# AiRyunn/BoT

Hardware: AMD Instinct MI355X
Metric: edges/sec full-batch GAT fwd+bwd on ogbn-arxiv; achieved HBM GB/s vs peak (higher is better)
Workload: dtype f32

## Files before the change

### bot_amd/_C.py

```python
from __future__ import annotations

import ctypes
import os
from ctypes import c_char_p, c_double, c_float, c_int32, c_int64, c_uint64, c_void_p

import torch

_HERE = os.path.dirname(os.path.abspath(__file__))
LIB_PATH = os.environ.get("BOT_AMD_LIB") or os.path.join(_HERE, "lib", "libbot_gnn.so")
ABI_VERSION = 19

if not os.path.exists(LIB_PATH):
    raise ImportError(
        f"{LIB_PATH} is missing: build the gfx950 kernels first "
        "(`make -C bot_amd/csrc` or `python -c 'import __graft_entry__ as g; g.build()'`). "
        "bot_amd has no CPU / PyTorch fallback."
    )
_lib = ctypes.CDLL(LIB_PATH)

_P = c_void_p
_SIGS = {
    "bot_abi_version": (ctypes.c_int, []),
    "bot_last_error": (c_char_p, []),
    "bot_last_kernel": (c_char_p, []),
# ... 32 lines not shown
    "bot_segment_sum_f32": (ctypes.c_int, [_P, c_int64, c_int64, _P, c_int64, c_int32, _P, _P, c_int32, _P, _P]),
    "bot_gather_rows_f32": (ctypes.c_int, [_P, c_int64, _P, c_int64, c_int32, _P, c_int64, _P]),
    "bot_scatter_add_rows_f32": (ctypes.c_int, [_P, c_int64, _P, c_int64, c_int32, _P, c_int64, _P]),
    "bot_merge_weight_fwd_f32": (ctypes.c_int, [_P, _P, _P, _P, c_int32, c_int32, c_int32, c_int32, c_int32, c_int32, _P, _P]),
    "bot_merge_weight_bwd_f32": (ctypes.c_int, [_P, _P, _P, c_int32, c_int32, c_int32, c_int32, c_int32, c_int32, _P, _P, _P, _P, _P, _P]),
    "bot_edge_mlp_workspace_floats": (c_int64, []),
    "bot_edge_mlp_fwd_f32": (ctypes.c_int, [_P, c_int32, _P, _P, c_int32, _P, c_int32, c_int64, _P, _P]),
    "bot_edge_mlp_bwd_f32": (ctypes.c_int, [_P, c_int32, _P, _P, c_int32, _P, c_int32, _P, c_int64, _P, _P, _P, _P, _P]),
    "bot_random_keep_workspace_bytes": (c_int64, []),
    "bot_random_keep_u8": (ctypes.c_int, [c_int64, c_int64, c_uint64, _P, _P, _P]),
    "bot_halves_workspace_floats": (c_int64, []),
    "bot_halves_scale_f32": (ctypes.c_int, [_P, c_int64, c_int64, c_int32, _P, _P, _P]),
    "bot_halves_split_f16": (ctypes.c_int, [_P, c_int64, c_int64, c_int32, _P, c_int32, _P, c_int64, c_int32, _P]),
    "bot_halves_split_cols_f16": (ctypes.c_int, [_P, c_int64, c_int64, c_int32, _P, c_int32, _P, c_int64, c_int32, c_int32, _P]),
    "bot_halves_split_heads_f16": (ctypes.c_int, [_P, c_int64, c_int64, c_int32, c_int32, _P, _P, c_int64, c_int32, c_int32, _P]),
    "bot_gemm_halves_f32": (ctypes.c_int, [c_int32, c_int32, c_int64, c_int64, c_int64, _P, _P, c_int64, _P, c_int64, _P, c_int64,
                                           c_int32, c_int64, c_int64, c_int64, c_float, _P, c_int64, c_int32, c_int32, _P]),
    "bot_gemm_halves3_nt_f32": (ctypes.c_int, [c_int64, c_int64, c_int64, _P, _P, _P, c_int64, c_int64, _P, c_int64, c_int64, _P, c_int64,
                                               c_int32, _P]),
    "bot_gemm_halves3_tn_workspace_floats": (c_int64, [c_int64, c_int64, c_int64]),
    "bot_gemm_halves3_tn_f32": (ctypes.c_int, [c_int64, c_int64, c_int64, c_int64, c_int64, _P, _P, _P, c_int64, c_int64, _P, c_int64, c_int64, _P,
                                               c_int64, _P, c_int32, _P]),
    "bot_gemm_halves3_nt_grouped_f32": (ctypes.c_int, [c_int64, c_int64, _P, _P, _P, c_int64, c_int64, _P, c_int64, c_int64, _P, c_int64, c_int32, _P,
                                                       c_int32, _P, _P, c_int32, _P, c_int32, _P]),
    "bot_gemm_halves3_tn_grouped_workspace_floats": (c_int64, [c_int64, c_int32]),
    "bot_gemm_halves3_tn_grouped_f32": (ctypes.c_int, [c_int64, _P, _P, _P, c_int64, c_int64, _P, c_int64, c_int64, _P, c_int32, _P, _P, c_int32, _P]),
    "bot_tn_narrow_workspace_floats": (c_int64, [c_int64, c_int32, c_int32]),
    "bot_tn_narrow_f32": (ctypes.c_int, [_P, c_int64, _P, c_int64, c_int64, c_int32, c_int32, _P, c_int64, c_int32, _P, _P]),
    "bot_bn_act_bwd_reduce_max_f32": (ctypes.c_int, [_P, c_int64, _P, c_int64, c_int64, c_int32, _P, _P, _P, _P, c_int32, c_float, c_uint64, _P, _P, _P, _P, _P]),
    "bot_bn_bwd_bound_f32": (ctypes.c_int, [c_int32, c_int64, _P, _P, _P, c_double, _P, _P, _P, _P]),
    "bot_bn_act_bwd_apply_halves_f32": (ctypes.c_int, [_P, c_int64, _P, c_int64, c_int64, c_int32, _P, _P, _P, _P, c_int32, c_float, c_uint64, _P, _P, _P, c_double,
                                                       _P, c_int64, _P, _P, c_int64, c_int32, c_int32, c_int32, _P]),
    "bot_label_split_f32": (ctypes.c_int, [_P, c_int64, _P, c_int64, _P, c_float, c_uint64, _P, c_int32, _P, _P, _P, _P, _P]),
    "bot_build_input_f32": (ctypes.c_int, [_P, c_int64, c_int64, c_int32, c_int32, _P, c_float, c_uint64, _P, _P, c_int64, _P]),
    "bot_node_loss_f32": (ctypes.c_int, [_P, c_int64, c_int64, c_int32, _P, c_int64, _P, _P, c_int32, c_float, _P, c_int64, _P, c_int64, _P]),
    "bot_rmsprop_step_f32": (ctypes.c_int, [c_int32, _P, _P, _P, _P, c_float, _P, c_float, c_float, c_float, _P]),
    "bot_gemm_halves_last_algo": (ctypes.c_int, [_P, _P]),
    "bot_gemm_halves_library_version": (ctypes.c_int, [_P, _P]),
    "bot_tn_gemm_workspace_floats": (c_int64, [c_int64, c_int32, c_int32, c_int32]),
    "bot_tn_gemm_f32": (ctypes.c_int, [_P, c_int64, _P, c_int64, c_int64, c_int32, c_int32, _P, c_int64, c_int32, c_int32, c_int64, c_int64,
                                       c_int64, _P, _P]),
    "bot_skinny_gemm_f32": (ctypes.c_int, [_P, c_int64, _P, c_int64, c_int32, _P, c_int64, c_int64, c_int32, c_int32, c_int32, c_int32,
                                           c_int64, c_int64, c_int64, _P]),
    "bot_bn_workspace_floats": (c_int64, [c_int32]),
    "bot_colstats_f32": (ctypes.c_int, [_P, c_int64, c_int64, c_int32, _P, _P, _P, _P]),
    "bot_colsum_f32": (ctypes.c_int, [_P, c_int64, c_int64, c_int32, _P, _P, _P]),
    "bot_bn_stats_f32": (ctypes.c_int, [_P, c_int64, c_int64, c_int32, c_float, c_float, _P, _P, _P, _P, _P, _P, _P]),
    "bot_bn_stats_halves_f32": (ctypes.c_int, [_P, c_int64, c_int64, c_int32, c_float, c_float, _P, _P, _P, _P, _P, _P, _P, c_float, _P, _P, _P]),
    "bot_bn_act_fwd_halves_f32": (ctypes.c_int, [_P, c_int64, c_int64, c_int32, _P, _P, _P, _P, c_int32, c_float, c_uint64, _P, _P, c_int64,
                                                 _P, _P, c_int64, c_int32, c_int32, _P]),
    "bot_bn_act_fwd_f32": (ctypes.c_int, [_P, c_int64, c_int64, c_int32, _P, _P, _P, _P, c_int32, c_float, c_uint64, _P, _P, c_int64, _P]),
    "bot_bn_act_bwd_reduce_f32": (ctypes.c_int, [_P, c_int64, _P, c_int64, c_int64, c_int32, _P, _P, _P, _P, c_int32, c_float,
                                                 c_uint64, _P, _P, _P, _P, _P]),
    "bot_bn_act_bwd_apply_f32": (ctypes.c_int, [_P, c_int64, _P, c_int64, c_int64, c_int32, _P, _P, _P, _P, c_int32, c_float,
                                                c_uint64, _P, _P, _P, c_double, _P, c_int64, _P, _P]),
    "bot_halves_tn_combine_f32": (ctypes.c_int, [_P, _P, c_int32, c_int32, c_int32, c_int32, _P, _P, _P, c_int64, _P]),
    "bot_halves_scale_from_slots2_f32": (ctypes.c_int, [_P, c_float, _P, c_float, _P, _P]),
    "bot_halves_tail_f16": (ctypes.c_int, [c_int64, c_int32, _P, _P, _P, _P, _P, c_int64, c_int32, _P]),
    "bot_spmm_dot_halves_fits": (ctypes.c_int, [_P, c_int64, c_int64, _P, c_int64, c_int64, c_int32, c_int32, _P, c_int64, c_int64, c_int32]),
    "bot_spmm_dot_halves_f16": (ctypes.c_int, [_P, _P, c_int64, c_int64, _P, c_int64, _P, _P, c_int64, _P, c_int64, c_int64, _P, _P, _P, c_int64, c_int64,
                                               c_int32, c_int32, _P, _P, c_int64, c_int64, c_int32, _P, _P, _P]),
    "bot_gemm_halves3_nt_bn_rows": (c_int32, [c_int64]),
    "bot_gemm_halves3_nt3_f32": (ctypes.c_int, [c_int64, c_int64, c_int64, _P, _P, c_int64, _P, _P, c_int64, c_int64, _P, c_int64, c_int64, c_int32, _P, c_int64,
                                                _P, c_int32, _P]),
    "bot_bn_act_bwd_reduce_partials_f32": (ctypes.c_int, [_P, c_int32, c_int32, _P, _P, _P]),
    "bot_bn_bwd_bound_partials_f32": (ctypes.c_int, [c_int32, _P, c_int32, _P, _P, c_double, _P, _P, _P, _P]),
    "bot_bn_bwd_partials_finish_f32": (ctypes.c_int, [_P, _P, c_int32, c_int32, _P, _P, c_int32, c_double, _P, _P, _P, _P]),
    "bot_gemm_halves3_nt2_f32": (ctypes.c_int, [c_int64, c_int64, c_int64, _P, _P, c_int64, _P, _P, c_int64, c_int64, _P, c_int64, c_int64, c_int32, _P, c_int64,
                                                c_int32, _P]),
    "bot_halves_split_frag_f16": (ctypes.c_int, [_P, c_int64, c_int64, c_int32, _P, _P, c_int32, _P]),
    "bot_gemm_halves3_tn2_f32": (ctypes.c_int, [c_int64, c_int64, c_int64, c_int64, c_int64, _P, _P, _P, c_int64, _P, c_int64, c_int64, _P, c_int64, c_int64, _P,
                                                c_int64, _P, c_int32, _P]),
    "bot_stream_create": (ctypes.c_int, [c_int32, _P]),
    "bot_gemm_halves3_nt_grouped2_f32": (ctypes.c_int, [c_int64, c_int64, _P, _P, _P, c_int64, c_int64, _P, c_int64, c_int64, _P, c_int64, c_int32, _P,
                                                        c_int32, _P, _P, c_int32, _P, _P, _P, _P, c_int32, c_int32, _P]),
    "bot_bn_stats_halves_partials_f32": (ctypes.c_int, [_P, _P, c_int32, _P, c_int64, c_int32, c_float, c_float, _P, _P, _P, _P, _P, _P, _P, c_float, _P, _P, _P]),
    "bot_absmax_slots": (c_int32, []),
    "bot_absmax_slots_f32": (ctypes.c_int, [_P, c_int64, c_int64, c_int32, _P, _P]),
    "bot_halves_scale_from_slots_f32": (ctypes.c_int, [_P, _P, _P]),
    "bot_sample_neighbors_count_i32": (ctypes.c_int, [_P, c_int64, _P, c_int64, c_int32, _P, _P]),
    "bot_sample_neighbors_i32": (ctypes.c_int, [_P, c_int64, _P, c_int64, c_int32, c_uint64, _P, _P, _P]),
    "bot_block_tiles": (c_int64, [c_int64]),
    "bot_block_mark_i32": (ctypes.c_int, [_P, c_int64, _P, _P, c_int64, _P, c_int64, _P, _P, _P]),
    "bot_block_relabel_i32": (ctypes.c_int, [_P, c_int64, _P, _P, _P, c_int64, _P, c_int64, _P, c_int64, _P, _P, _P, _P]),
}
for _name, (_res, _args) in _SIGS.items():
    _fn = getattr(_lib, _name)
    _fn.restype, _fn.argtypes = _res, _args
EXPORTED = tuple(_SIGS)

if _lib.bot_abi_version() != ABI_VERSION:
    raise ImportError(f"libbot_gnn.so ABI {_lib.bot_abi_version()} != binding ABI {ABI_VERSION}; rebuild")


class BotKernelError(RuntimeError):
    pass


PROFILE = None


PROFILE_SKIP = ()


def _timed(name, key, launch):
    if PROFILE is None or name in PROFILE_SKIP:
# ... 986 lines not shown
        y = torch.empty((n, F), dtype=torch.float32, device=x.device) if want_y else None
        buf = torch.empty((n, pieces * piece), dtype=torch.float16, device=x.device)
        _check(_timed("bn_act_fwd", (F,), lambda: _lib.bot_bn_act_fwd_halves_f32(
            x.data_ptr(), x.stride(0), n, F, mean.data_ptr(), invstd.data_ptr(), _ptr(weight), _ptr(bias), int(relu), float(p),
            int(seed), _seed_off(p), _ptr(y), F, hscale.data_ptr(), buf.data_ptr(), buf.stride(0), piece, pieces, _stream())),
            "bn_act_fwd_halves")
        return y, buf
    y = torch.empty((n, F), dtype=torch.float32, device=x.device)
    _check(_timed("bn_act_fwd", (F,), lambda: _lib.bot_bn_act_fwd_f32(
        x.data_ptr(), x.stride(0), n, F, mean.data_ptr(), invstd.data_ptr(), _ptr(weight), _ptr(bias), int(relu), float(p),
        int(seed), _seed_off(p), y.data_ptr(), y.stride(0), _stream())), "bn_act_fwd")
    return y


def bn_act_bwd_reduce(dy, x, mean, invstd, weight, bias, relu, p, seed, want_max=False):
    _dev(dy, x)
    dy, x = _mat(dy, "dy"), _mat(x, "x")
    n, F = x.shape
    sg = torch.empty(F, dtype=torch.float32, device=x.device)
    sgx = torch.empty(F, dtype=torch.float32, device=x.device)
    ws = _bn_ws(F, x.device)
    fn = _lib.bot_bn_act_bwd_reduce_max_f32 if want_max else _lib.bot_bn_act_bwd_reduce_f32
    _check(fn(dy.data_ptr(), dy.stride(0), x.data_ptr(), x.stride(0), n, F, mean.data_ptr(), invstd.data_ptr(), _ptr(weight), _ptr(bias), int(relu),
              float(p), int(seed), _seed_off(p), sg.data_ptr(), sgx.data_ptr(), ws.data_ptr(), _stream()), "bn_act_bwd_reduce")
    return (sg, sgx, ws) if want_max else (sg, sgx)


def bn_bwd_bound(ws, n, sum_g, sum_gx, total_count, weight, invstd, slots):
    _dev(ws, invstd, slots)
    F = invstd.shape[0]
    _check(_lib.bot_bn_bwd_bound_f32(F, n, ws.data_ptr(), _ptr(sum_g), _ptr(sum_gx), float(total_count), _ptr(weight), invstd.data_ptr(), slots.data_ptr(),
                                     _stream()), "bn_bwd_bound")
    return slots


def bn_act_bwd_apply_halves(dy, x, mean, invstd, weight, bias, relu, p, seed, sum_g, sum_gx, total_count, hscale, hout, hD, hDP, out=None, h2_off=None):
    _dev(dy, x, hout, hscale)
    dy, x = _mat(dy, "dy"), _mat(x, "x")
    n, F = x.shape
    if h2_off is None:
        h2_off = (F // hD) * hDP
        assert hout.shape == (n, 2 * h2_off)
    else:
        assert hout.shape[0] == n and hout.stride(0) >= h2_off + (F // hD) * hDP
    assert hout.dtype == torch.float16 and hout.stride(1) == 1
    assert out is None or (out.stride(1) == 1 and out.dtype == torch.float32)
    _check(_lib.bot_bn_act_bwd_apply_halves_f32(dy.data_ptr(), dy.stride(0), x.data_ptr(), x.stride(0), n, F, mean.data_ptr(), invstd.data_ptr(), _ptr(weight),
                                                _ptr(bias), int(relu), float(p), int(seed), _seed_off(p), _ptr(sum_g), _ptr(sum_gx), float(total_count),
                                                _ptr(out), out.stride(0) if out is not None else 0, hscale.data_ptr(), hout.data_ptr(), hout.stride(0), h2_off,
                                                hD, hDP, _stream()), "bn_act_bwd_apply_halves")
    return hout


def bn_act_bwd_apply(dy, x, mean, invstd, weight, bias, relu, p, seed, sum_g, sum_gx, total_count, out=None, absmax=None):
    _dev(dy, x)
    dy, x = _mat(dy, "dy"), _mat(x, "x")
    n, F = x.shape
    dx = out if out is not None else torch.empty((n, F), dtype=torch.float32, device=x.device)
    assert dx.stride(1) == 1 and dx.dtype == torch.float32
    _check(_lib.bot_bn_act_bwd_apply_f32(dy.data_ptr(), dy.stride(0), x.data_ptr(), x.stride(0), n, F, mean.data_ptr(),
                                         invstd.data_ptr(), _ptr(weight), _ptr(bias), int(relu), float(p), int(seed), _seed_off(p),
                                         _ptr(sum_g), _ptr(sum_gx), float(total_count), dx.data_ptr(), dx.stride(0), _ptr(absmax),
                                         _stream()),
           "bn_act_bwd_apply")
    return dx


def edge_mlp_supported(I, J, H):
    return I == 8 and J == 16 and 1 <= H <= 8


def random_keep(n, n_keep, seed, device):
    device = torch.device(device)
    if device.type != "cuda":
        raise BotKernelError("random_keep: the HIP kernels need a GPU device")
    keep = torch.empty(n, dtype=torch.uint8, device=device)
    ws = torch.empty(int(_lib.bot_random_keep_workspace_bytes()), dtype=torch.uint8, device=device)
    with torch.cuda.device(device):
        _check(_lib.bot_random_keep_u8(n, n_keep, seed & 0xFFFFFFFFFFFFFFFF, keep.data_ptr(), ws.data_ptr(), _stream()), "random_keep")
    return keep


def sample_neighbors(csc, seeds, k, seed):
    _dev(csc.indptr, seeds)
    assert seeds.dtype == torch.int32 and seeds.is_contiguous()
    n = int(seeds.numel())
    dev = seeds.device
    counts = torch.empty(n, dtype=torch.int32, device=dev)
    _check(_lib.bot_sample_neighbors_count_i32(csc.indptr.data_ptr(), csc.n_rows, _ptr(seeds), n, int(k), _ptr(counts), _stream()),
           "sample_neighbors_count")
    offsets = torch.zeros(n + 1, dtype=torch.int64, device=dev)
    torch.cumsum(counts, 0, out=offsets[1:])
    total = int(offsets[-1])
    pos = torch.empty(total, dtype=torch.int32, device=dev)
    _check(_timed("sample", (int(k),), lambda: _lib.bot_sample_neighbors_i32(
        csc.indptr.data_ptr(), csc.n_rows, _ptr(seeds), n, int(k), seed & 0xFFFFFFFFFFFFFFFF, offsets.data_ptr(), _ptr(pos), _stream())),
        "sample_neighbors")
    return offsets, pos


def block_relabel(csc, seeds, pos, node_map):
    _dev(csc.indptr, seeds, pos, node_map)
    n_seeds, n_pos, n_nodes = int(seeds.numel()), int(pos.numel()), int(node_map.numel())
    dev = seeds.device
    tiles = torch.empty(max(1, int(_lib.bot_block_tiles(n_nodes))), dtype=torch.int64, device=dev)
    n_new = torch.zeros(1, dtype=torch.int64, device=dev)
# ... 61 lines not shown
```

### bot_amd/csrc/dense.hip

```cpp
#include <hip/hip_fp16.h>

#include "common.h"

#include <stdlib.h>

namespace bot {

constexpr int kTX = 64;
constexpr int kTY = 4;
constexpr int kRowBlocks = 256;

template <int VEC>
__device__ __forceinline__ void drop_factors(uint64_t seed, int64_t r, int c, int64_t nquad, float p, float scale, float (&f)[VEC]) {
    uint32_t w[4];
    Philox::gen(seed, (uint64_t)(r * nquad + (c >> 2)), w);
#pragma unroll
    for (int t = 0; t < VEC; ++t) f[t] = ((w[(c & 3) + t] >> 8) * (1.0f / 16777216.0f)) >= p ? scale : 0.f;
}

template <int VEC>
__device__ __forceinline__ void load_cols(float (&v)[VEC], const float* p, bool wide, int nv) {
    if constexpr (VEC == 4) {
        if (wide && nv == 4) {
            vload<4>(v, p);
        } else {
            const float2 a = *reinterpret_cast<const float2*>(p);
            v[0] = a.x, v[1] = a.y, v[2] = 0.f, v[3] = 0.f;
            if (nv == 4) {
                const float2 b = *reinterpret_cast<const float2*>(p + 2);
                v[2] = b.x, v[3] = b.y;
            }
        }
    } else {
        vload<VEC>(v, p);
    }
}
template <int VEC>
__device__ __forceinline__ void store_cols(float* p, const float (&v)[VEC], bool wide, int nv) {
    if constexpr (VEC == 4) {
        if (wide && nv == 4) {
            vstore<4>(p, v);
        } else {
            *reinterpret_cast<float2*>(p) = make_float2(v[0], v[1]);
            if (nv == 4) *reinterpret_cast<float2*>(p + 2) = make_float2(v[2], v[3]);
        }
    } else {
        vstore<VEC>(p, v);
    }
}
template <int VEC>
__device__ __forceinline__ void load_param(float (&v)[VEC], const float* a, int c, int F, float dflt) {
#pragma unroll
    for (int t = 0; t < VEC; ++t) v[t] = (a && c + t < F) ? a[c + t] : dflt;
}

__device__ __forceinline__ uint64_t eff_seed(uint64_t seed, const uint64_t* off) {
    return off ? seed + off[0] * 0x9E3779B97F4A7C15ull : seed;
// ... 534 lines not shown
#pragma unroll
        for (int g = 1; g < kWideGroups; ++g) gm = fmaxf(gm, lds[0][g][lc]), xm = fmaxf(xm, lds[1][g][lc]);
        float t = gm;
        if (sum_g) t += fabsf(sum_g[c]) * inv_count + xm * fabsf(sum_gx[c]) * inv_count;
        b = fabsf(w ? w[c] : 1.f) * invstd[c] * t * 1.0001f;
    }
    if (threadIdx.x < 64) absmax_publish(wave_absmax(b), slots);
}

__global__ __launch_bounds__(kWideCols * kWideGroups) void bn_bwd_finish_wide_kernel(int32_t F, const float* part, const float* pmax, int nblk, float* s0, float* s1,
                                                                                    float inv_count, bool batch_stats, const float* w, const float* invstd,
                                                                                    uint32_t* slots) {
    __shared__ double lds[2][kWideGroups][kWideCols];
    __shared__ float ldm[2][kWideGroups][kWideCols];
    const int lc = threadIdx.x % kWideCols, c = blockIdx.x * kWideCols + lc, grp = threadIdx.x / kWideCols;
    double s = 0.0, q = 0.0;
    float gm = 0.f, xm = 0.f;
    if (c < F) {
        int b = grp;
        for (; b + 3 * kWideGroups < nblk; b += 4 * kWideGroups) {
            float vs[4], vq[4], vg[4], vx[4];
#pragma unroll
            for (int j = 0; j < 4; ++j) {
                const int64_t o = ((int64_t)(b + kWideGroups * j) * 2) * F + c;
                vs[j] = part[o], vq[j] = part[o + F], vg[j] = pmax[o], vx[j] = pmax[o + F];
            }
#pragma unroll
            for (int j = 0; j < 4; ++j) s += (double)vs[j], q += (double)vq[j], gm = fmaxf(gm, vg[j]), xm = fmaxf(xm, vx[j]);
        }
        for (; b < nblk; b += kWideGroups) {
            const int64_t o = ((int64_t)b * 2) * F + c;
            s += (double)part[o], q += (double)part[o + F], gm = fmaxf(gm, pmax[o]), xm = fmaxf(xm, pmax[o + F]);
        }
    }
    lds[0][grp][lc] = s, lds[1][grp][lc] = q, ldm[0][grp][lc] = gm, ldm[1][grp][lc] = xm;
    __syncthreads();
    float bnd = 0.f;
    if (grp == 0 && c < F) {
        double S = 0.0, Q = 0.0;
#pragma unroll
        for (int g = 0; g < kWideGroups; ++g) S += lds[0][g][lc], Q += lds[1][g][lc];
#pragma unroll
        for (int g = 1; g < kWideGroups; ++g) gm = fmaxf(gm, ldm[0][g][lc]), xm = fmaxf(xm, ldm[1][g][lc]);
        const float fs = (float)S, fq = (float)Q;
        s0[c] = fs, s1[c] = fq;
        float t = gm;
        if (batch_stats) t += fabsf(fs) * inv_count + xm * fabsf(fq) * inv_count;
        bnd = fabsf(w ? w[c] : 1.f) * invstd[c] * t * 1.0001f;
    }
    if (threadIdx.x < 64) absmax_publish(wave_absmax(bnd), slots);
}

template <int VEC>
__global__ __launch_bounds__(kTX* kTY) void bn_act_bwd_apply_kernel(BnArgs a) {
    const int tx = threadIdx.x % kTX, ty = threadIdx.x / kTX;
    const int c = (blockIdx.x * kTX + tx) * VEC;
    float amax = 0.f;
    if (c < a.F) {
        const int nv = min(VEC, a.F - c);
        float mu[VEC], is[VEC], sc[VEC], sh[VEC], mg[VEC], mgx[VEC];
        load_param<VEC>(mu, a.mean, c, a.F, 0.f);
        load_param<VEC>(is, a.invstd, c, a.F, 0.f);
        load_param<VEC>(sc, a.w, c, a.F, 1.f);
        load_param<VEC>(sh, a.b, c, a.F, 0.f);
        load_param<VEC>(mg, a.sum_g, c, a.F, 0.f);
        load_param<VEC>(mgx, a.sum_gx, c, a.F, 0.f);
#pragma unroll
        for (int t = 0; t < VEC; ++t) mg[t] *= a.inv_count, mgx[t] *= a.inv_count;
        const float scale = a.p > 0.f ? 1.f / (1.f - a.p) : 1.f;
        const int64_t nquad = (a.F + 3) / 4;
        const uint64_t seed = eff_seed(a.seed, a.seed_offset);
        constexpr int UR = 4;
        const int64_t step = (int64_t)gridDim.y * kTY;
        int hdst[(VEC + 1) / 2] = {};
        bool hquad = false;
        const float hs = a.hout ? a.hscale[0] : 1.f;
        if (a.hout) {
#pragma unroll
            for (int t = 0; t < VEC; t += 2) {
                const int cc = c + t, hd = cc / a.hD;
                hdst[t / 2] = hd * a.hDP + (cc - hd * a.hD);
            }
            if constexpr (VEC == 4) hquad = nv == 4 && c / a.hD == (c + 3) / a.hD;
        }
        for (int64_t r0 = (int64_t)blockIdx.y * kTY + ty; r0 < a.n; r0 += step * UR) {
            float v[UR][VEC], g[UR][VEC];
#pragma unroll
            for (int u = 0; u < UR; ++u) {
                const int64_t r = r0 + u * step;
                if (r < a.n) {
                    load_cols<VEC>(v[u], a.x + r * a.ldx + c, a.wx, nv);
                    load_cols<VEC>(g[u], a.dy + r * a.lddy + c, a.wdy, nv);
                }
            }
#pragma unroll
            for (int u = 0; u < UR; ++u) {
                const int64_t r = r0 + u * step;
                if (r >= a.n) break;
                float f[VEC];
                if (a.p > 0.f) drop_factors<VEC>(seed, r, c, nquad, a.p, scale, f);
#pragma unroll
                for (int t = 0; t < VEC; ++t) {
                    const float xh = (v[u][t] - mu[t]) * is[t];
                    float gg = g[u][t];
                    if (a.p > 0.f) gg *= f[t];
                    if (a.relu && !(fmaf(xh, sc[t], sh[t]) > 0.f)) gg = 0.f;
                    v[u][t] = sc[t] * is[t] * (gg - mg[t] - xh * mgx[t]);
                    if (t < nv) amax = fmaxf(amax, fabsf(v[u][t]));
                }
                if (a.dx) store_cols<VEC>(a.dx + r * a.lddx + c, v[u], a.wdx, nv);
                if (a.hout) {
                    __half* ho = a.hout + r * a.ldh;
                    __half h1[VEC], h2[VEC];
#pragma unroll
                    for (int t = 0; t < VEC; ++t) {
                        const float z = (t < nv ? v[u][t] : 0.f) * hs;
                        h1[t] = __float2half_rn(z);
                        h2[t] = __float2half_rn((z - __half2float(h1[t])) * kHalvesShift);
                    }
                    if constexpr (VEC == 4) {
                        if (hquad) {
                            *reinterpret_cast<uint2*>(ho + hdst[0]) = *reinterpret_cast<const uint2*>(h1);
                            *reinterpret_cast<uint2*>(ho + hdst[0] + a.h2off) = *reinterpret_cast<const uint2*>(h2);
                            continue;
                        }
                    }
#pragma unroll
                    for (int t = 0; t < VEC; t += 2) {
                        if (t >= nv) break;
                        if (VEC >= 2 && t + 1 < nv) {
                            *reinterpret_cast<__half2*>(ho + hdst[t / 2]) = __halves2half2(h1[t], h1[t + 1]);
                            *reinterpret_cast<__half2*>(ho + hdst[t / 2] + a.h2off) = __halves2half2(h2[t], h2[t + 1]);
                        } else {
                            ho[hdst[t / 2]] = h1[t], ho[hdst[t / 2] + a.h2off] = h2[t];
                        }
                    }
                }
            }
        }
    }
    if (a.absmax) absmax_publish(wave_absmax(amax), a.absmax);
}

static inline bool rows16(const void* p, int64_t ld) { return p != nullptr && aligned(p, 16) && ld % 4 == 0; }
static int bn_vec(int32_t F, std::initializer_list<int64_t> strides, std::initializer_list<const void*> ptrs, bool* quad) {
    const int v = pick_vec(F, strides, ptrs);
    *quad = false;
    if (v == 4 || F % 2 != 0) return v;
    for (int64_t st : strides)
        if (st % 2 != 0) return v;
    for (const void* p : ptrs)
        if (p != nullptr && !aligned(p, 8)) return v;
    *quad = true;
    return 4;
}

static dim3 bn_grid(int32_t F, int vec, int64_t n) {
    const int64_t rb = (n + kTY - 1) / kTY;
    return dim3((unsigned)((F + kTX * vec - 1) / (kTX * vec)), (unsigned)(rb < kRowBlocks ? (rb > 0 ? rb : 1) : kRowBlocks));
}

}

extern "C" {

int64_t bot_bn_workspace_floats(int32_t F) { return (int64_t)bot::kRowBlocks * 4 * F + F; }

int bot_colstats_f32(const float* x, int64_t ldx, int64_t n, int32_t F, float* mean, float* m2, float* workspace,
                     bot_stream_t stream) {
    using namespace bot;
    BOT_REQUIRE(n >= 1 && F >= 1 && ldx >= F, BOT_E_RANGE, "colstats: n=%lld F=%d ldx=%lld", (long long)n, F, (long long)ldx);
    BOT_REQUIRE(x && mean && m2 && workspace, BOT_E_NULL, "colstats: NULL pointer");
    hipStream_t st = (hipStream_t)stream;
    bool quad;
    const int vec = bn_vec(F, {ldx}, {x}, &quad);
    const bool wx = !quad || rows16(x, ldx);
    const dim3 grid = bn_grid(F, vec, n);
    if (vec == 4) hipLaunchKernelGGL((colstats_partial_kernel<4>), grid, dim3(kTX * kTY), 0, st, x, ldx, n, F, workspace, wx, true);
    else if (vec == 2) hipLaunchKernelGGL((colstats_partial_kernel<2>), grid, dim3(kTX * kTY), 0, st, x, ldx, n, F, workspace, true, true);
    else hipLaunchKernelGGL((colstats_partial_kernel<1>), grid, dim3(kTX * kTY), 0, st, x, ldx, n, F, workspace, true, true);
    hipLaunchKernelGGL(colstats_final_kernel, dim3((F + 63) / 64), dim3(kBlock), 0, st, x, n, F, workspace, (int)grid.y,
                       mean, m2, (float*)nullptr, 0.f, 0.f, (float*)nullptr, (float*)nullptr, (int64_t*)nullptr);
    return hip_status("colstats launch");
}

int bot_colsum_f32(const float* x, int64_t ldx, int64_t n, int32_t F, float* sum, float* workspace, bot_stream_t stream) {
    using namespace bot;
    BOT_REQUIRE(n >= 1 && F >= 1 && ldx >= F, BOT_E_RANGE, "colsum: n=%lld F=%d ldx=%lld", (long long)n, F, (long long)ldx);
    BOT_REQUIRE(x && sum && workspace, BOT_E_NULL, "colsum: NULL pointer");
    hipStream_t st = (hipStream_t)stream;
    bool quad;
    const int vec = bn_vec(F, {ldx}, {x}, &quad);
    const bool wx = !quad || rows16(x, ldx);
    const dim3 grid = bn_grid(F, vec, n);
    if (vec == 4) hipLaunchKernelGGL((colstats_partial_kernel<4>), grid, dim3(kTX * kTY), 0, st, x, ldx, n, F, workspace, wx, false);
    else if (vec == 2) hipLaunchKernelGGL((colstats_partial_kernel<2>), grid, dim3(kTX * kTY), 0, st, x, ldx, n, F, workspace, true, false);
    else hipLaunchKernelGGL((colstats_partial_kernel<1>), grid, dim3(kTX * kTY), 0, st, x, ldx, n, F, workspace, true, false);
    hipLaunchKernelGGL(colsum_final_kernel, dim3((F + 63) / 64), dim3(kBlock), 0, st, workspace, F, (int)grid.y, sum);
    return hip_status("colsum launch");
}

int bot_bn_stats_f32(const float* x, int64_t ldx, int64_t n, int32_t F, float eps, float momentum, float* mean, float* invstd,
                     float* running_mean, float* running_var, int64_t* num_batches_tracked, float* workspace,
                     bot_stream_t stream) {
    using namespace bot;
    BOT_REQUIRE(n >= 1 && F >= 1 && ldx >= F, BOT_E_RANGE, "bn_stats: n=%lld F=%d ldx=%lld", (long long)n, F, (long long)ldx);
    BOT_REQUIRE(x && mean && invstd && workspace, BOT_E_NULL, "bn_stats: NULL pointer");
    BOT_REQUIRE((running_mean == nullptr) == (running_var == nullptr), BOT_E_NULL, "bn_stats: running_mean and running_var go together");
    BOT_REQUIRE(eps >= 0.f && momentum >= 0.f && momentum <= 1.f, BOT_E_RANGE, "bn_stats: eps=%f momentum=%f", (double)eps, (double)momentum);
    hipStream_t st = (hipStream_t)stream;
    bool quad;
    const int vec = bn_vec(F, {ldx}, {x}, &quad);
    const bool wx = !quad || rows16(x, ldx);
    const dim3 grid = bn_grid(F, vec, n);
    if (vec == 4) hipLaunchKernelGGL((colstats_partial_kernel<4>), grid, dim3(kTX * kTY), 0, st, x, ldx, n, F, workspace, wx, true);
    else if (vec == 2) hipLaunchKernelGGL((colstats_partial_kernel<2>), grid, dim3(kTX * kTY), 0, st, x, ldx, n, F, workspace, true, true);
    else hipLaunchKernelGGL((colstats_partial_kernel<1>), grid, dim3(kTX * kTY), 0, st, x, ldx, n, F, workspace, true, true);
// ... 174 lines not shown
    hipLaunchKernelGGL(pair_final_kernel, dim3((F + 63) / 64), dim3(kBlock), 0, st, F, workspace, (int)grid.y, sum_g,
                       sum_gx);
    return hip_status("bn_act_bwd_reduce launch");
}

static int bn_act_bwd_apply_impl(const float* dy, int64_t lddy, const float* x, int64_t ldx, int64_t n, int32_t F, const float* mean, const float* invstd,
                                 const float* weight, const float* bias, int32_t relu, float p, uint64_t seed, const uint64_t* seed_offset, const float* sum_g,
                                 const float* sum_gx, double total_count, float* dx, int64_t lddx, uint32_t* absmax_slots, const float* hscale, uint16_t* hout,
                                 int64_t ldh, int32_t h2_off, int32_t hD, int32_t hDP, bot_stream_t stream);

int bot_bn_act_bwd_apply_f32(const float* dy, int64_t lddy, const float* x, int64_t ldx, int64_t n, int32_t F,
                             const float* mean, const float* invstd, const float* weight, const float* bias, int32_t relu,
                             float p, uint64_t seed, const uint64_t* seed_offset, const float* sum_g, const float* sum_gx,
                             double total_count, float* dx, int64_t lddx, uint32_t* absmax_slots, bot_stream_t stream) {
    BOT_REQUIRE(dx || n == 0, BOT_E_NULL, "bn_act_bwd_apply: NULL pointer");
    return bn_act_bwd_apply_impl(dy, lddy, x, ldx, n, F, mean, invstd, weight, bias, relu, p, seed, seed_offset, sum_g, sum_gx, total_count, dx, lddx,
                                 absmax_slots, nullptr, nullptr, 0, 0, 0, 0, stream);
}

int bot_bn_act_bwd_apply_halves_f32(const float* dy, int64_t lddy, const float* x, int64_t ldx, int64_t n, int32_t F, const float* mean, const float* invstd,
                                    const float* weight, const float* bias, int32_t relu, float p, uint64_t seed, const uint64_t* seed_offset,
                                    const float* sum_g, const float* sum_gx, double total_count, float* dx, int64_t lddx, const float* hscale, uint16_t* hout,
                                    int64_t ldh, int32_t h2_off, int32_t hD, int32_t hDP, bot_stream_t stream) {
    using namespace bot;
    BOT_REQUIRE(hscale && hout, BOT_E_NULL, "bn_act_bwd_apply_halves: NULL pointer");
    BOT_REQUIRE(hD >= 2 && hD % 2 == 0 && hDP >= hD && hDP % 2 == 0 && F % hD == 0 && h2_off % 2 == 0 && ldh % 2 == 0 && h2_off >= (int64_t)(F / hD) * hDP &&
                    ldh >= h2_off + (int64_t)(F / hD) * hDP && aligned(hout, 4), BOT_E_RANGE, "bn_act_bwd_apply_halves: F=%d hD=%d hDP=%d h2_off=%d ldh=%lld", F, hD, hDP,
                h2_off, (long long)ldh);
    return bn_act_bwd_apply_impl(dy, lddy, x, ldx, n, F, mean, invstd, weight, bias, relu, p, seed, seed_offset, sum_g, sum_gx, total_count, dx, lddx, nullptr,
                                 hscale, hout, ldh, h2_off, hD, hDP, stream);
}

static int bn_act_bwd_apply_impl(const float* dy, int64_t lddy, const float* x, int64_t ldx, int64_t n, int32_t F, const float* mean, const float* invstd,
                                 const float* weight, const float* bias, int32_t relu, float p, uint64_t seed, const uint64_t* seed_offset, const float* sum_g,
                                 const float* sum_gx, double total_count, float* dx, int64_t lddx, uint32_t* absmax_slots, const float* hscale, uint16_t* hout,
                                 int64_t ldh, int32_t h2_off, int32_t hD, int32_t hDP, bot_stream_t stream) {
    using namespace bot;
    BOT_REQUIRE(n >= 0 && F >= 1 && ldx >= F && lddy >= F && (dx == nullptr || lddx >= F), BOT_E_RANGE, "bn_act_bwd_apply: n=%lld F=%d", (long long)n, F);
    if (n == 0) return 0;
    BOT_REQUIRE(dy && x && mean && invstd && (dx || hout), BOT_E_NULL, "bn_act_bwd_apply: NULL pointer");
    BOT_REQUIRE((sum_g == nullptr) == (sum_gx == nullptr), BOT_E_NULL, "bn_act_bwd_apply: sum_g and sum_gx go together");
    BOT_REQUIRE(sum_g == nullptr || total_count >= 1.0, BOT_E_RANGE, "bn_act_bwd_apply: total_count=%f", total_count);
    BnArgs a{};
    a.x = x, a.ldx = ldx, a.n = n, a.F = F, a.mean = mean, a.invstd = invstd, a.w = weight, a.b = bias, a.relu = relu, a.p = p;
    a.seed = seed, a.seed_offset = seed_offset, a.dy = dy, a.lddy = lddy, a.sum_g = sum_g, a.sum_gx = sum_gx, a.inv_count = sum_g ? (float)(1.0 / total_count) : 0.f;
    a.dx = dx, a.lddx = lddx, a.absmax = absmax_slots;
    a.hout = reinterpret_cast<__half*>(hout), a.hscale = hscale, a.ldh = ldh, a.h2off = h2_off, a.hD = hD, a.hDP = hDP;
    if (!dx) lddx = ldx;
    bool quad;
    const int vec = bn_vec(F, {ldx, lddy, lddx}, {x, dy, dx}, &quad);
    a.wx = !quad || rows16(x, ldx), a.wdy = !quad || rows16(dy, lddy), a.wdx = !quad || rows16(dx, lddx);
    const dim3 grid = bn_grid(F, vec, n);
    hipStream_t st = (hipStream_t)stream;
    if (vec == 4) hipLaunchKernelGGL((bn_act_bwd_apply_kernel<4>), grid, dim3(kTX * kTY), 0, st, a);
    else if (vec == 2) hipLaunchKernelGGL((bn_act_bwd_apply_kernel<2>), grid, dim3(kTX * kTY), 0, st, a);
    else hipLaunchKernelGGL((bn_act_bwd_apply_kernel<1>), grid, dim3(kTX * kTY), 0, st, a);
    return hip_status("bn_act_bwd_apply launch");
}

}
```

### include/bot_gnn.h

```cpp
#ifndef BOT_GNN_H
#define BOT_GNN_H

#include <stdint.h>

#ifdef __cplusplus
extern "C" {
#endif

#define BOT_ABI_VERSION 19

#define BOT_E_NULL (-1)
#define BOT_E_RANGE (-2)
#define BOT_E_ALIGN (-3)
#define BOT_E_PLAN (-4)

typedef void* bot_stream_t;

int bot_abi_version(void);
const char* bot_last_error(void);
int bot_stream_create(int32_t high_priority, bot_stream_t* out);
const char* bot_last_kernel(void);
int bot_debug_abort_trace(const char* path_host);

int bot_row_plan_size_host(const int32_t* indptr_host, int64_t n_rows, int32_t chunk,
// ... 93 lines not shown
                      const float* el, int64_t ldel, const float* er, int64_t lder,
                      const float* ee, const float* ew, float slope, int32_t H, int32_t D,
                      const float* addend, int64_t lda, int64_t hsa,
                      const float* scale, const float* shift, int32_t relu,
                      float* out, int64_t ldo, int64_t hso,
                      float* workspace, uint32_t* absmax_slots , bot_stream_t stream);

int bot_segment_sum_f32(const int32_t* indptr, int64_t n_rows, int64_t nnz,
                        const int32_t* long_rows, int64_t n_long, int32_t chunk,
                        const float* vals, const int32_t* perm, int32_t W,
                        float* out, bot_stream_t stream);

int bot_gather_rows_f32(const float* x, int64_t ldx, const int32_t* rows, int64_t n_sel, int32_t F,
                        float* out, int64_t ldo, bot_stream_t stream);
int bot_scatter_add_rows_f32(float* x, int64_t ldx, const int32_t* rows, int64_t n_sel, int32_t F,
                             const float* vals, int64_t ldv, bot_stream_t stream);

int64_t bot_bn_workspace_floats(int32_t F);
int bot_colstats_f32(const float* x, int64_t ldx, int64_t n, int32_t F, float* mean, float* m2, float* workspace,
                     bot_stream_t stream);
int bot_colsum_f32(const float* x, int64_t ldx, int64_t n, int32_t F, float* sum, float* workspace, bot_stream_t stream);
int bot_bn_stats_f32(const float* x, int64_t ldx, int64_t n, int32_t F, float eps, float momentum, float* mean, float* invstd,
                     float* running_mean, float* running_var, int64_t* num_batches_tracked, float* workspace,
                     bot_stream_t stream);
int bot_bn_act_fwd_f32(const float* x, int64_t ldx, int64_t n, int32_t F, const float* mean, const float* invstd,
                       const float* weight, const float* bias, int32_t relu, float p, uint64_t seed,
                       const uint64_t* seed_offset, float* y, int64_t ldy, bot_stream_t stream);
int bot_bn_stats_halves_f32(const float* x, int64_t ldx, int64_t n, int32_t F, float eps, float momentum, float* mean, float* invstd,
                            float* running_mean, float* running_var, int64_t* num_batches_tracked, const float* weight,
                            const float* bias, float p, float* hscale, float* workspace, bot_stream_t stream);
int bot_bn_act_fwd_halves_f32(const float* x, int64_t ldx, int64_t n, int32_t F, const float* mean, const float* invstd,
                              const float* weight, const float* bias, int32_t relu, float p, uint64_t seed,
                              const uint64_t* seed_offset, float* y, int64_t ldy, const float* hscale, uint16_t* hout, int64_t ldh,
                              int32_t piece, int32_t pieces, bot_stream_t stream);
int bot_bn_act_bwd_reduce_f32(const float* dy, int64_t lddy, const float* x, int64_t ldx, int64_t n, int32_t F,
                              const float* mean, const float* invstd, const float* weight, const float* bias,
                              int32_t relu, float p, uint64_t seed, const uint64_t* seed_offset, float* sum_g, float* sum_gx,
                              float* workspace, bot_stream_t stream);
int bot_bn_act_bwd_apply_f32(const float* dy, int64_t lddy, const float* x, int64_t ldx, int64_t n, int32_t F,
                             const float* mean, const float* invstd, const float* weight, const float* bias,
                             int32_t relu, float p, uint64_t seed, const uint64_t* seed_offset, const float* sum_g,
                             const float* sum_gx, double total_count, float* dx, int64_t lddx, uint32_t* absmax_slots , bot_stream_t stream);
int bot_bn_act_bwd_reduce_max_f32(const float* dy, int64_t lddy, const float* x, int64_t ldx, int64_t n, int32_t F,
                                  const float* mean, const float* invstd, const float* weight, const float* bias,
                                  int32_t relu, float p, uint64_t seed, const uint64_t* seed_offset, float* sum_g, float* sum_gx,
                                  float* workspace, bot_stream_t stream);
int bot_bn_bwd_bound_f32(int32_t F, int64_t n, const float* workspace, const float* sum_g, const float* sum_gx, double total_count,
                         const float* weight, const float* invstd, uint32_t* absmax_slots, bot_stream_t stream);
int bot_bn_act_bwd_apply_halves_f32(const float* dy, int64_t lddy, const float* x, int64_t ldx, int64_t n, int32_t F,
                                    const float* mean, const float* invstd, const float* weight, const float* bias,
                                    int32_t relu, float p, uint64_t seed, const uint64_t* seed_offset, const float* sum_g,
                                    const float* sum_gx, double total_count, float* dx, int64_t lddx, const float* hscale, uint16_t* hout,
                                    int64_t ldh, int32_t h2_off, int32_t hD, int32_t hDP, bot_stream_t stream);

int bot_merge_weight_fwd_f32(const float* W, const float* Wres, const float* attn_l, const float* attn_r, int32_t H, int32_t D,
                             int32_t K, int32_t P, int32_t with_fc, int32_t block, float* merged, bot_stream_t stream);
int bot_merge_weight_bwd_f32(const float* W, const float* attn_l, const float* attn_r, int32_t H, int32_t D, int32_t K,
                             int32_t P, int32_t with_fc, int32_t block, const float* d_merged, float* dW, float* dWres,
                             float* d_attn_l, float* d_attn_r, bot_stream_t stream);

int64_t bot_edge_mlp_workspace_floats(void);
int bot_edge_mlp_fwd_f32(const float* ef, int32_t I, const float* W1, const float* b1, int32_t J, const float* W2,
                         int32_t H, int64_t n_edges, float* ee, bot_stream_t stream);
int bot_edge_mlp_bwd_f32(const float* ef, int32_t I, const float* W1, const float* b1, int32_t J, const float* W2,
                         int32_t H, const float* dz, int64_t n_edges, float* dW1, float* db1, float* dW2,
                         float* workspace, bot_stream_t stream);

int64_t bot_random_keep_workspace_bytes(void);
int bot_random_keep_u8(int64_t n, int64_t n_keep, uint64_t seed, uint8_t* keep, void* workspace, bot_stream_t stream);

int bot_sample_neighbors_count_i32(const int32_t* indptr, int64_t n_rows, const int32_t* seeds, int64_t n_seeds, int32_t k, int32_t* counts,
                                   bot_stream_t stream);
int bot_sample_neighbors_i32(const int32_t* indptr, int64_t n_rows, const int32_t* seeds, int64_t n_seeds, int32_t k, uint64_t seed,
                             const int64_t* offsets, int32_t* out, bot_stream_t stream);
int64_t bot_block_tiles(int64_t n_nodes);
int bot_block_mark_i32(const int32_t* seeds, int64_t n_seeds, const int32_t* indices, const int32_t* pos, int64_t n_pos, int32_t* map,
                       int64_t n_nodes, int64_t* tile_counts, int64_t* n_new, bot_stream_t stream);
int bot_block_relabel_i32(const int32_t* seeds, int64_t n_seeds, const int32_t* indices, const int32_t* eid, const int32_t* pos, int64_t n_pos,
                          int32_t* map, int64_t n_nodes, const int64_t* tile_offsets, int64_t n_src, int32_t* src_nid, int32_t* local,
                          int32_t* parent_eid, bot_stream_t stream);

int64_t bot_halves_workspace_floats(void);
int bot_halves_scale_f32(const float* x, int64_t ldx, int64_t n, int32_t F, float* scale, float* workspace, bot_stream_t stream);
int32_t bot_absmax_slots(void);
int bot_absmax_slots_f32(const float* x, int64_t ldx, int64_t n, int32_t F, uint32_t* slots, bot_stream_t stream);
int bot_halves_scale_from_slots_f32(const uint32_t* slots, float* scale, bot_stream_t stream);
int bot_halves_split_f16(const float* x, int64_t ldx, int64_t n, int32_t F, const float* scale, int32_t order, uint16_t* out,
                         int64_t ldo, int32_t piece, bot_stream_t stream);
int bot_halves_split_cols_f16(const float* x, int64_t ldx, int64_t n, int32_t F, const float* scale, int32_t order, uint16_t* out,
                              int64_t ldo, int32_t piece, int32_t width, bot_stream_t stream);
int bot_halves_split_heads_f16(const float* x, int64_t ldx, int64_t n, int32_t H, int32_t D, const float* scale, uint16_t* out, int64_t ldo,
                               int32_t h2_off, int32_t DP, bot_stream_t stream);
int bot_halves_tn_combine_f32(const float* a, const float* b, int32_t chunks, int32_t K, int32_t PP, int32_t P, const float* rem_a,
                              const float* rem_b, float* out, int64_t ldo, bot_stream_t stream);
int bot_gemm_halves_f32(int32_t trans_a, int32_t trans_b, int64_t m, int64_t n, int64_t k, const float* alpha, const uint16_t* A,
                        int64_t lda, const uint16_t* B, int64_t ldb, float* C, int64_t ldc, int32_t batch, int64_t stride_a,
                        int64_t stride_b, int64_t stride_c, float beta, void* workspace, int64_t workspace_bytes, int32_t tune,
                        int32_t algo_index, bot_stream_t stream);
int bot_gemm_halves3_nt_f32(int64_t m, int64_t n, int64_t k, const float* scale_a, const float* scale_b, const uint16_t* A, int64_t lda,
                            int64_t a2_off, const uint16_t* B, int64_t ldb, int64_t b2_off, float* C, int64_t ldc, int32_t mode,
                            bot_stream_t stream);
int64_t bot_gemm_halves3_tn_workspace_floats(int64_t n_rows, int64_t kp, int64_t pp);
int bot_gemm_halves3_tn_f32(int64_t n_rows, int64_t k, int64_t p, int64_t kp, int64_t pp, const float* scale_x, const float* scale_d,
                            const uint16_t* X, int64_t ldx, int64_t x2_off, const uint16_t* D, int64_t ldd, int64_t d2_off, float* out,
                            int64_t ldo, float* workspace, int32_t mode, bot_stream_t stream);

// ... 87 lines not shown
```

Before: 241.3 million.

## Add row-segment launch for BN backward apply with one block per row group

Pulls the per-column parameter setup and per-row math of the BN+activation backward apply into a shared helper. Adds a row-segment kernel in which each 256-thread block covers the whole feature width for a fixed group of rows (default 8), loading all of those rows before computing. The new path is on by default for vec4 with F up to 1024, and an environment variable or API call can choose the row count. It replaces the grid-stride loop, whose grid is capped at a fixed number of row blocks, with many small blocks, aiming for more memory parallelism. In exchange, each block reloads the column parameters, and the arithmetic order changes slightly (fmaf, contract off).

```diff
diff --git a/bot_amd/_C.py b/bot_amd/_C.py
--- a/bot_amd/_C.py
+++ b/bot_amd/_C.py
@@ -108,6 +108,7 @@
     "bot_bn_act_fwd_f32": (ctypes.c_int, [_P, c_int64, c_int64, c_int32, _P, _P, _P, _P, c_int32, c_float, c_uint64, _P, _P, c_int64, _P]),
     "bot_bn_act_bwd_reduce_f32": (ctypes.c_int, [_P, c_int64, _P, c_int64, c_int64, c_int32, _P, _P, _P, _P, c_int32, c_float,
                                                  c_uint64, _P, _P, _P, _P, _P]),
+    "bot_bn_bwd_apply_rows": (c_int32, [c_int32]),
     "bot_bn_act_bwd_apply_f32": (ctypes.c_int, [_P, c_int64, _P, c_int64, c_int64, c_int32, _P, _P, _P, _P, c_int32, c_float,
                                                 c_uint64, _P, _P, _P, c_double, _P, c_int64, _P, _P]),
     "bot_halves_tn_combine_f32": (ctypes.c_int, [_P, _P, c_int32, c_int32, c_int32, c_int32, _P, _P, _P, c_int64, _P]),
@@ -1200,6 +1201,12 @@
     return hout
 
 
+def bn_bwd_apply_rows(rows=None):
+    r = _lib.bot_bn_bwd_apply_rows(-1 if rows is None else int(rows))
+    _check(min(r, 0), "bn_bwd_apply_rows")
+    return r
+
+
 def bn_act_bwd_apply(dy, x, mean, invstd, weight, bias, relu, p, seed, sum_g, sum_gx, total_count, out=None, absmax=None):
     _dev(dy, x)
     dy, x = _mat(dy, "dy"), _mat(x, "x")
diff --git a/bot_amd/csrc/dense.hip b/bot_amd/csrc/dense.hip
--- a/bot_amd/csrc/dense.hip
+++ b/bot_amd/csrc/dense.hip
@@ -3,6 +3,8 @@
 #include "common.h"
 
 #include <stdlib.h>
+
+#include <atomic>
 
 namespace bot {
 
@@ -643,37 +645,92 @@
 }
 
 template <int VEC>
+struct BwdApplyCols {
+    int c, nv;
+    float mu[VEC], is[VEC], sc[VEC], sh[VEC], mg[VEC], mgx[VEC];
+    float scale, hs;
+    int64_t nquad;
+    uint64_t seed;
+    int hdst[(VEC + 1) / 2];
+    bool hquad;
+
+    __device__ __forceinline__ BwdApplyCols(const BnArgs& a, int c_) : c(c_), nv(min(VEC, a.F - c_)), hdst{}, hquad(false) {
+        load_param<VEC>(mu, a.mean, c, a.F, 0.f);
+        load_param<VEC>(is, a.invstd, c, a.F, 0.f);
+        load_param<VEC>(sc, a.w, c, a.F, 1.f);
+        load_param<VEC>(sh, a.b, c, a.F, 0.f);
+        load_param<VEC>(mg, a.sum_g, c, a.F, 0.f);
+        load_param<VEC>(mgx, a.sum_gx, c, a.F, 0.f);
+#pragma unroll
+        for (int t = 0; t < VEC; ++t) mg[t] *= a.inv_count, mgx[t] *= a.inv_count;
+        scale = a.p > 0.f ? 1.f / (1.f - a.p) : 1.f;
+        nquad = (a.F + 3) / 4;
+        seed = eff_seed(a.seed, a.seed_offset);
+        hs = a.hout ? a.hscale[0] : 1.f;
+        if (a.hout) {
+#pragma unroll
+            for (int t = 0; t < VEC; t += 2) {
+                const int cc = c + t, hd = cc / a.hD;
+                hdst[t / 2] = hd * a.hDP + (cc - hd * a.hD);
+            }
+            if constexpr (VEC == 4) hquad = nv == 4 && c / a.hD == (c + 3) / a.hD;
+        }
+    }
+
+    __device__ __forceinline__ void row(const BnArgs& a, int64_t r, float (&v)[VEC], const float (&g)[VEC], float& amax) const {
+#pragma clang fp contract(off)
+        float f[VEC];
+        if (a.p > 0.f) drop_factors<VEC>(seed, r, c, nquad, a.p, scale, f);
+#pragma unroll
+        for (int t = 0; t < VEC; ++t) {
+            const float xh = (v[t] - mu[t]) * is[t];
+            float gg = g[t];
+            if (a.p > 0.f) gg *= f[t];
+            if (a.relu && !(fmaf(xh, sc[t], sh[t]) > 0.f)) gg = 0.f;
+            v[t] = sc[t] * is[t] * fmaf(-xh, mgx[t], gg - mg[t]);
+            if (t < nv) amax = fmaxf(amax, fabsf(v[t]));
+        }
+        if (a.dx) store_cols<VEC>(a.dx + r * a.lddx + c, v, a.wdx, nv);
+        if (a.hout) {
+            __half* ho = a.hout + r * a.ldh;
+            __half h1[VEC], h2[VEC];
+#pragma unroll
+            for (int t = 0; t < VEC; ++t) {
+                const float z = (t < nv ? v[t] : 0.f) * hs + 0.f;
+                h1[t] = __float2half_rn(z);
+                h2[t] = __float2half_rn((z - __half2float(h1[t])) * kHalvesShift);
+            }
+            if constexpr (VEC == 4) {
+                if (hquad) {
+                    *reinterpret_cast<uint2*>(ho + hdst[0]) = *reinterpret_cast<const uint2*>(h1);
+                    *reinterpret_cast<uint2*>(ho + hdst[0] + a.h2off) = *reinterpret_cast<const uint2*>(h2);
+                    return;
+                }
+            }
+#pragma unroll
+            for (int t = 0; t < VEC; t += 2) {
+                if (t >= nv) break;
+                if (VEC >= 2 && t + 1 < nv) {
+                    *reinterpret_cast<__half2*>(ho + hdst[t / 2]) = __halves2half2(h1[t], h1[t + 1]);
+                    *reinterpret_cast<__half2*>(ho + hdst[t / 2] + a.h2off) = __halves2half2(h2[t], h2[t + 1]);
+                } else {
+                    ho[hdst[t / 2]] = h1[t], ho[hdst[t / 2] + a.h2off] = h2[t];
+                }
+            }
+        }
+    }
+};
+
+template <int VEC>
 __global__ __launch_bounds__(kTX* kTY) void bn_act_bwd_apply_kernel(BnArgs a) {
     const int tx = threadIdx.x % kTX, ty = threadIdx.x / kTX;
     const int c = (blockIdx.x * kTX + tx) * VEC;
     float amax = 0.f;
     if (c < a.F) {
         const int nv = min(VEC, a.F - c);
-        float mu[VEC], is[VEC], sc[VEC], sh[VEC], mg[VEC], mgx[VEC];
-        load_param<VEC>(mu, a.mean, c, a.F, 0.f);
-        load_param<VEC>(is, a.invstd, c, a.F, 0.f);
-        load_param<VEC>(sc, a.w, c, a.F, 1.f);
-        load_param<VEC>(sh, a.b, c, a.F, 0.f);
-        load_param<VEC>(mg, a.sum_g, c, a.F, 0.f);
-        load_param<VEC>(mgx, a.sum_gx, c, a.F, 0.f);
-#pragma unroll
-        for (int t = 0; t < VEC; ++t) mg[t] *= a.inv_count, mgx[t] *= a.inv_count;
-        const float scale = a.p > 0.f ? 1.f / (1.f - a.p) : 1.f;
-        const int64_t nquad = (a.F + 3) / 4;
-        const uint64_t seed = eff_seed(a.seed, a.seed_offset);
+        const BwdApplyCols<VEC> cols(a, c);
         constexpr int UR = 4;
         const int64_t step = (int64_t)gridDim.y * kTY;
-        int hdst[(VEC + 1) / 2] = {};
-        bool hquad = false;
-        const float hs = a.hout ? a.hscale[0] : 1.f;
-        if (a.hout) {
-#pragma unroll
-            for (int t = 0; t < VEC; t += 2) {
-                const int cc = c + t, hd = cc / a.hD;
-                hdst[t / 2] = hd * a.hDP + (cc - hd * a.hD);
-            }
-            if constexpr (VEC == 4) hquad = nv == 4 && c / a.hD == (c + 3) / a.hD;
-        }
         for (int64_t r0 = (int64_t)blockIdx.y * kTY + ty; r0 < a.n; r0 += step * UR) {
             float v[UR][VEC], g[UR][VEC];
 #pragma unroll
@@ -688,46 +745,32 @@
             for (int u = 0; u < UR; ++u) {
                 const int64_t r = r0 + u * step;
                 if (r >= a.n) break;
-                float f[VEC];
-                if (a.p > 0.f) drop_factors<VEC>(seed, r, c, nquad, a.p, scale, f);
-#pragma unroll
-                for (int t = 0; t < VEC; ++t) {
-                    const float xh = (v[u][t] - mu[t]) * is[t];
-                    float gg = g[u][t];
-                    if (a.p > 0.f) gg *= f[t];
-                    if (a.relu && !(fmaf(xh, sc[t], sh[t]) > 0.f)) gg = 0.f;
-                    v[u][t] = sc[t] * is[t] * (gg - mg[t] - xh * mgx[t]);
-                    if (t < nv) amax = fmaxf(amax, fabsf(v[u][t]));
-                }
-                if (a.dx) store_cols<VEC>(a.dx + r * a.lddx + c, v[u], a.wdx, nv);
-                if (a.hout) {
-                    __half* ho = a.hout + r * a.ldh;
-                    __half h1[VEC], h2[VEC];
-#pragma unroll
-                    for (int t = 0; t < VEC; ++t) {
-                        const float z = (t < nv ? v[u][t] : 0.f) * hs;
-                        h1[t] = __float2half_rn(z);
-                        h2[t] = __float2half_rn((z - __half2float(h1[t])) * kHalvesShift);
-                    }
-                    if constexpr (VEC == 4) {
-                        if (hquad) {
-                            *reinterpret_cast<uint2*>(ho + hdst[0]) = *reinterpret_cast<const uint2*>(h1);
-                            *reinterpret_cast<uint2*>(ho + hdst[0] + a.h2off) = *reinterpret_cast<const uint2*>(h2);
-                            continue;
-                        }
-                    }
-#pragma unroll
-                    for (int t = 0; t < VEC; t += 2) {
-                        if (t >= nv) break;
-                        if (VEC >= 2 && t + 1 < nv) {
-                            *reinterpret_cast<__half2*>(ho + hdst[t / 2]) = __halves2half2(h1[t], h1[t + 1]);
-                            *reinterpret_cast<__half2*>(ho + hdst[t / 2] + a.h2off) = __halves2half2(h2[t], h2[t + 1]);
-                        } else {
-                            ho[hdst[t / 2]] = h1[t], ho[hdst[t / 2] + a.h2off] = h2[t];
-                        }
-                    }
-                }
-            }
+                cols.row(a, r, v[u], g[u], amax);
+            }
+        }
+    }
+    if (a.absmax) absmax_publish(wave_absmax(amax), a.absmax);
+}
+
+template <int R>
+__global__ __launch_bounds__(256) void bn_act_bwd_apply_rowseg_kernel(BnArgs a) {
+    const int c = threadIdx.x * 4;
+    float amax = 0.f;
+    if (c < a.F) {
+        const int nv = min(4, a.F - c);
+        const BwdApplyCols<4> cols(a, c);
+        const int64_t r0 = (int64_t)blockIdx.x * R;
+        float v[R][4], g[R][4];
+#pragma unroll
+        for (int u = 0; u < R; ++u)
+            if (r0 + u < a.n) {
+                load_cols<4>(v[u], a.x + (r0 + u) * a.ldx + c, a.wx, nv);
+                load_cols<4>(g[u], a.dy + (r0 + u) * a.lddy + c, a.wdy, nv);
+            }
+#pragma unroll
+        for (int u = 0; u < R; ++u) {
+            if (r0 + u >= a.n) break;
+            cols.row(a, r0 + u, v[u], g[u], amax);
         }
     }
     if (a.absmax) absmax_publish(wave_absmax(amax), a.absmax);
@@ -746,6 +789,14 @@
     return 4;
 }
 
+constexpr int kBwdRowSeg = 8;
+static bool bwd_rows_ok(int r) { return r == 0 || r == 2 || r == 4 || r == 8 || r == 16; }
+static std::atomic<int> bwd_apply_rows{[] {
+    const char* e = getenv("BOT_BN_BWD_ROWSEG");
+    const int r = e && *e ? atoi(e) : kBwdRowSeg;
+    return bwd_rows_ok(r) ? r : kBwdRowSeg;
+}()};
+
 static dim3 bn_grid(int32_t F, int vec, int64_t n) {
     const int64_t rb = (n + kTY - 1) / kTY;
     return dim3((unsigned)((F + kTX * vec - 1) / (kTX * vec)), (unsigned)(rb < kRowBlocks ? (rb > 0 ? rb : 1) : kRowBlocks));
@@ -754,6 +805,13 @@
 }
 
 extern "C" {
+
+int32_t bot_bn_bwd_apply_rows(int32_t rows) {
+    using namespace bot;
+    if (rows < 0) return bwd_apply_rows.load();
+    BOT_REQUIRE(bwd_rows_ok(rows), BOT_E_RANGE, "bn_bwd_apply_rows: %d is not 0, 2, 4, 8 or 16", rows);
+    return bwd_apply_rows.exchange(rows);
+}
 
 int64_t bot_bn_workspace_floats(int32_t F) { return (int64_t)bot::kRowBlocks * 4 * F + F; }
 
@@ -1034,6 +1092,15 @@
     a.wx = !quad || rows16(x, ldx), a.wdy = !quad || rows16(dy, lddy), a.wdx = !quad || rows16(dx, lddx);
     const dim3 grid = bn_grid(F, vec, n);
     hipStream_t st = (hipStream_t)stream;
+    const int rows = bwd_apply_rows.load(std::memory_order_relaxed);
+    if (vec == 4 && F <= 1024 && rows > 0) {
+        const dim3 rgrid((unsigned)((n + rows - 1) / rows)), rblock((unsigned)(((F + 3) / 4 + 63) / 64 * 64));
+        if (rows == 2) hipLaunchKernelGGL((bn_act_bwd_apply_rowseg_kernel<2>), rgrid, rblock, 0, st, a);
+        else if (rows == 4) hipLaunchKernelGGL((bn_act_bwd_apply_rowseg_kernel<4>), rgrid, rblock, 0, st, a);
+        else if (rows == 8) hipLaunchKernelGGL((bn_act_bwd_apply_rowseg_kernel<8>), rgrid, rblock, 0, st, a);
+        else hipLaunchKernelGGL((bn_act_bwd_apply_rowseg_kernel<16>), rgrid, rblock, 0, st, a);
+        return hip_status("bn_act_bwd_apply rowseg launch");
+    }
     if (vec == 4) hipLaunchKernelGGL((bn_act_bwd_apply_kernel<4>), grid, dim3(kTX * kTY), 0, st, a);
     else if (vec == 2) hipLaunchKernelGGL((bn_act_bwd_apply_kernel<2>), grid, dim3(kTX * kTY), 0, st, a);
     else hipLaunchKernelGGL((bn_act_bwd_apply_kernel<1>), grid, dim3(kTX * kTY), 0, st, a);
diff --git a/include/bot_gnn.h b/include/bot_gnn.h
--- a/include/bot_gnn.h
+++ b/include/bot_gnn.h
@@ -169,6 +169,7 @@
                                     int32_t relu, float p, uint64_t seed, const uint64_t* seed_offset, const float* sum_g,
                                     const float* sum_gx, double total_count, float* dx, int64_t lddx, const float* hscale, uint16_t* hout,
                                     int64_t ldh, int32_t h2_off, int32_t hD, int32_t hDP, bot_stream_t stream);
+int32_t bot_bn_bwd_apply_rows(int32_t rows);
 
 int bot_merge_weight_fwd_f32(const float* W, const float* Wres, const float* attn_l, const float* attn_r, int32_t H, int32_t D,
                              int32_t K, int32_t P, int32_t with_fc, int32_t block, float* merged, bot_stream_t stream);
```

Result: no change. 240.9 million, median of 6 (-0.2%).
